# ToughStoneX/Self-Supervised-MVS

Hardware: AMD Instinct MI355X
Metric: depth-samples/sec (N=3, 640x512, D=192) (higher is better)
Workload: dtype f32

## Files before the change

### self-supervised-mvs_amd/_lib.py

```python
from __future__ import annotations

import contextlib
import ctypes as C
import os

_HERE = os.path.dirname(os.path.abspath(__file__))
LIB_PATH = os.path.join(_HERE, "libmvs_hip.so")

_f = C.c_void_p
_i = C.c_int
_ll = C.c_longlong
_s = C.c_void_p
_fl = C.c_float

class MvsUnetBlock(C.Structure):
    _fields_ = [("transposed", _i), ("stride", _i), ("src", _i), ("skip", _i), ("eps", _fl), ("momentum", _fl),
                ("cin", _i), ("cout", _i), ("d", _i), ("h", _i), ("w", _i)]


class MvsFeatBlock(C.Structure):
    _fields_ = [("cin", _i), ("cout", _i), ("ks", _i), ("stride", _i), ("eps", _fl), ("momentum", _fl), ("w_channels_last", _i),
                ("h", _i), ("w", _i)]


# ... 110 lines not shown
    "mvs_maxpool2x2_cl": (_i, [_f, _f, _i, _i, _i, _i, _s]),
    "mvs_resize_bilinear_cl": (_i, [_f, _f, _i, _i, _i, _i, _i, _i, _s]),
    "mvs_conv_trunk_fwd": (_i, [_i, C.POINTER(MvsTrunkLayer), _pp, _pp, _f, _f, _f, _f, _f, _i, _i, _i, _s]),
    "mvs_conv2d_wide_packed_bytes_arith": (_ll, [_i, _i, _i]),
    "mvs_conv2d_wide_workspace_floats_arith": (_ll, [_i] * 6),
    "mvs_conv2d_wide_pack_weights_arith": (_i, [_f, _f, _i, _i, _i, _i, _s]),
    "mvs_conv2d_wide_fwd_arith": (_i, [_f, _f, _f, _f, _f, _i, _i, _i, _i, _i, _i, _i, _i, _s]),
    "mvs_conv_trunk_fwd_arith": (_i, [_i, C.POINTER(MvsTrunkLayer), _pp, _pp, _f, _f, _f, _f, _f, _i, _i, _i, _i, _s]),
}

OP_CONV_FWD, OP_CONV_DGRAD, OP_CONV_WGRAD, OP_CONVT_FWD, OP_CONVT_DGRAD, OP_CONVT_WGRAD = range(6)


class MvsLib:

    def __init__(self, path: str = LIB_PATH, device_type: str = "cuda"):
        if not os.path.exists(path):
            raise RuntimeError(
                "libmvs_hip.so not found at %s -- build it with `python __graft_entry__.py` "
                "(hipcc --offload-arch=gfx950); there is no CPU / PyTorch fallback for the hot path" % path)
        self.path = path
        self.device_type = device_type
        self.cdll = C.CDLL(path)
        self.profiler = None
        for name, (res, args) in SIGNATURES.items():
            fn = getattr(self.cdll, name)
            fn.restype = res
            fn.argtypes = args
            setattr(self, "_" + name, fn)

    def call(self, name: str, *args, tag="", tstream=None):
        prof = self.profiler
        if prof is not None and (prof.names is None or name in prof.names):
            if not isinstance(tag, str):
                tag = tag[0] % tuple(tag[1:])
            if prof.wants(name, tag):
                import torch
                ev0, ev1 = torch.cuda.Event(enable_timing=True), torch.cuda.Event(enable_timing=True)
                ev0.record(tstream)
                rc = getattr(self, "_" + name)(*args)
                ev1.record(tstream)
                prof.add(name, tag, ev0, ev1)
                if rc != 0:
                    self._raise(name, rc)
                return
        rc = getattr(self, "_" + name)(*args)
        if rc != 0:
            self._raise(name, rc)

    def _raise(self, name, rc):
        msg = self._mvs_last_error().decode("utf-8", "replace")
        if rc in (-1, -2, -4):
            raise ValueError("%s failed (%d): %s" % (name, rc, msg))
        raise RuntimeError("%s failed (%d): %s" % (name, rc, msg))

    def raw(self, name: str, *args):
        return getattr(self, "_" + name)(*args)

    def launch_trace(self):
        buf = C.create_string_buffer(4096)
        self._mvs_launch_trace(buf, len(buf))
        return [s for s in buf.value.decode().split(",") if s]

    def get_tuning(self, key: str) -> int:
        v = _i()
        self.call("mvs_get_tuning", key.encode(), C.byref(v))
        return v.value

    @contextlib.contextmanager
    def tuning(self, **knobs):
        old = []
        try:
            for key, val in knobs.items():
                old.append((key, self.get_tuning(key)))
                self.call("mvs_set_tuning", key.encode(), int(val))
            yield self
        finally:
            for key, val in reversed(old):
                self.call("mvs_set_tuning", key.encode(), val)


_INSTANCE = None

DEFAULT_TUNING = {"k8": 7, "xcd": 1, "side_pre": 1, "conv_pers": 1, "conv_pers_min": 1024, "conv_pers_nw": 8, "wgrad_pers": 1, "conv_small": 1, "tr2pw": 1, "sweep_bwd": 0, "wgrad_small": 0, "wgrad_groups": 768, "wgrad8_groups": 192, "wgrad8_gs": 2, "wgrad8_nch": 2, "cout1_h4": 1, "wgrad2d_batch": 2048, "sweep_fwd": 3}


def get() -> MvsLib:
    global _INSTANCE
    if _INSTANCE is None:
        _INSTANCE = MvsLib()
        for item in filter(None, os.environ.get("MVS_TUNING", "").split(",")):
            key, _, val = item.partition("=")
            DEFAULT_TUNING[key.strip()] = int(val)
            _INSTANCE.call("mvs_set_tuning", key.strip().encode(), int(val))
    return _INSTANCE


class KernelTimer:

    def __init__(self, only=None, names=None):
        self.only = only
        self.names = names
        self.events = {}

    def wants(self, name, tag):
        return self.only is None or name in self.only or tag in self.only

    def add(self, name, tag, ev0, ev1):
        self.events.setdefault((name, tag), []).append((ev0, ev1))

    _REG_NAMES = frozenset(("mvs_conv3d_fwd", "mvs_convT3d_fwd", "mvs_conv3d_dgrad", "mvs_convT3d_dgrad", "mvs_conv3d_wgrad", "mvs_convT3d_wgrad",
                            "mvs_bn_relu_fwd_slots", "mvs_bn_relu_bwd_slots", "mvs_bn_bwd_reduce_slots", "mvs_conv3d_pack_weights_batch"))

    def allows_c_entry(self, lib, blocks):
        if self.names is None:
            return False
        hit = self.names & self._REG_NAMES
        if not hit:
            return True
        if not hit <= {"mvs_conv3d_wgrad", "mvs_convT3d_wgrad"} or self.only is None:
            return False
        want = [t for t in self.only if isinstance(t, str) and t.startswith("wgrad")]
        found = []
        for i, (transposed, cin, cout, stride, dims) in enumerate(blocks):
            tag = "%s:%d>%d:s%d:%dx%dx%dx%d" % (("wgradT" if transposed else "wgrad", cin, cout, stride) + tuple(dims))
            if tag in want:
                found.append((i, "mvs_convT3d_wgrad" if transposed else "mvs_conv3d_wgrad", tag))
        if len(found) != 1 or len(want) != 1:
            return False
        owner = getattr(lib, "_unet_timer", None)
        if owner is not self:
            if owner is not None:
                owner._harvest()
                owner._c = None
            lib.raw("mvs_unet_time_read", (C.c_float * 1024)(), 1024)
            lib.raw("mvs_unet_time_wgrad", found[0][0])
            lib._unet_timer = self
            self._c = (lib, found[0])
        return True

    def _harvest(self):
        c = getattr(self, "_c", None)
        if c is None:
            return
        lib, (idx, name, tag) = c
        buf = (C.c_float * 1024)()
        cnt = lib.raw("mvs_unet_time_read", buf, 1024)
        if cnt > 0:
            acc = self.__dict__.setdefault("_c_acc", {})
            n0, s0 = acc.get((name, tag), (0, 0.0))
            acc[(name, tag)] = (n0 + cnt, s0 + sum(buf[:cnt]))

    def release_c_bracket(self, lib):
        self._harvest()
        self._c = None
        lib.raw("mvs_unet_time_wgrad", -2)
        lib._unet_timer = None

    def summary(self):
        out = {}
        for k, evs in self.events.items():
            ms = [a.elapsed_time(b) for a, b in evs]
            out[k] = (len(ms), sum(ms) / len(ms))
        c = getattr(self, "_c", None)
        if c is not None:
            self.release_c_bracket(c[0])
        for (name, tag), (cnt, tot) in getattr(self, "_c_acc", {}).items():
# ... 7 lines not shown
```

### self-supervised-mvs_amd/csrc/conv3d.hip

```cpp
#include "mvs_rt.h"
#include "conv_map.h"

#include "conv_args.h"

__device__ __forceinline__ void conv_pack_weights_item(const float* __restrict__ w, float* __restrict__ wp, int geom, int CC,
                                                       int Cin, int Cout, int NB, int layout, int flip, int idx) {
    const int j = idx & 3, lane = (idx >> 2) & 63;
    const int nb = (idx >> 8) % NB, kk = (idx >> 8) / NB;
    const int co = nb * 16 + (lane & 15);
    int ks, chunk = 0, cls = 0;
    if (geom == GEOM_TR2_PW) {
        int k0 = 0;
        for (cls = 0; cls < 4; ++cls) {
            int n = tr2p_ntaps(cls) * CC / 16;
            if (kk < k0 + n) break;
            k0 += n;
        }
        ks = kk - k0;
        const int kf = 16 * ks + 4 * (lane >> 4) + j;
        const int tp = kf / CC, cip = kf % CC, n = lane & 15, pw = n >> 3, cop = n & 7;
        int dd, dh, dw, kd, kh;
        tr2p_tap(cls, tp, dd, dh, dw, kd, kh);
        int kw = tr2p_kw(pw, dw);
        float v = 0.f;
// ... 968 lines not shown
                acc[p][0] = mfma_4x4x1_bc(w0, x4.x, acc[p][0], 4 * cq + 0);
                acc[p][1] = mfma_4x4x1_bc(w1, x4.x, acc[p][1], 4 * cq + 0);
                acc[p][0] = mfma_4x4x1_bc(w0, x4.y, acc[p][0], 4 * cq + 1);
                acc[p][1] = mfma_4x4x1_bc(w1, x4.y, acc[p][1], 4 * cq + 1);
                acc[p][0] = mfma_4x4x1_bc(w0, x4.z, acc[p][0], 4 * cq + 2);
                acc[p][1] = mfma_4x4x1_bc(w1, x4.z, acc[p][1], 4 * cq + 2);
                acc[p][0] = mfma_4x4x1_bc(w0, x4.w, acc[p][0], 4 * cq + 3);
                acc[p][1] = mfma_4x4x1_bc(w1, x4.w, acc[p][1], 4 * cq + 3);
            }
        }
    }
    const int qd = qd0 + wave, qh = qh0 + (lane >> 4), qw = qw0 + (lane & 15);
    const bool inside = qd < a.QD && qh < a.QH && qw < a.QW;
#pragma unroll
    for (int h = 0; h < 2; ++h) {
        float o[4];
#pragma unroll
        for (int r = 0; r < 4; ++r) {
            const int co = 4 * h + r;
            float val = acc[0][h][r] + acc[1][h][r];
            if (!inside || co >= a.Cout) val = 0.f;
            s1[co] += val;
            s2[co] += val * val;
            if (co < a.Cout) {
                if (a.scale) val = val * a.scale[co] + a.shift[co];
                else if (a.shift) val = val + a.shift[co];
                if (a.relu) val = fmaxf(val, 0.f);
            }
            o[r] = val;
        }
        if (inside) {
            const size_t obase = ((((size_t)b * a.Do + qd) * a.Ho + qh) * a.Wo + qw) * a.Cout + 4 * h;
            if (a.Cout == 8) {
                float4 ov = make_float4(o[0], o[1], o[2], o[3]);
                if (a.skip) {
                    const float4 sk = *reinterpret_cast<const float4*>(a.skip + obase);
                    ov.x += sk.x; ov.y += sk.y; ov.z += sk.z; ov.w += sk.w;
                }
                *reinterpret_cast<float4*>(a.y + obase) = ov;
            } else {
#pragma unroll
                for (int r = 0; r < 4; ++r)
                    if (4 * h + r < a.Cout) a.y[obase + r] = o[r] + (a.skip ? a.skip[obase + r] : 0.f);
            }
        }
    }
    }
    if (a.slots) {
        float v[16];
#pragma unroll
        for (int c = 0; c < 8; ++c) { v[c] = s1[c]; v[8 + c] = s2[c]; }
#define MVS_BFLY_STEP(N, M)                                              \
        {                                                                \
            const bool up = (lane & (M)) != 0;                           \
            _Pragma("unroll") for (int q = 0; q < (N); ++q) {            \
                const float keep = up ? v[(N) + q] : v[q];               \
                const float send = up ? v[q] : v[(N) + q];               \
                v[q] = keep + __shfl_xor(send, (M));                     \
            }                                                            \
        }
        MVS_BFLY_STEP(8, 32)
        MVS_BFLY_STEP(4, 16)
        MVS_BFLY_STEP(2, 8)
        MVS_BFLY_STEP(1, 4)
#undef MVS_BFLY_STEP
        float r = v[0];
        r += __shfl_xor(r, 2);
        r += __shfl_xor(r, 1);
        if ((lane & 3) == 0) {
            const int idx = ((lane >> 5) & 1) * 8 + ((lane >> 4) & 1) * 4 + ((lane >> 3) & 1) * 2 + ((lane >> 2) & 1);
            red[wave * 16 + idx] = r;
        }
        __syncthreads();
        if (tid < 16) {
            const int stat = tid >> 3, co = tid & 7;
            if (co < a.Cout)
                MVS_GLOBAL_ATOMIC_ADD_F64(a.slots + ((size_t)(blockIdx.x & (a.nslots - 1)) * 2 + stat) * a.Cout + co,
                                          (double)(red[tid] + red[16 + tid] + red[32 + tid] + red[48 + tid]));
        }
    }
}


template <bool BC, int NCH>
__global__ __launch_bounds__(256) void conv_c8_wgrad_kernel(WgradArgs a) {
    using G = ConvGeom<GEOM_S1>;
    constexpr int CC = 16, CCP = 16;
    constexpr int RHP = 7, RWP = 19;
    constexpr int NRP = G::RD * RHP * RWP;
    constexpr int NPOS = G::TQD * G::TQH * G::TQW;
    constexpr int NTG = 7;
    __shared__ __attribute__((aligned(16))) float xt[NCH * NRP * CCP];
    __shared__ __attribute__((aligned(16))) float gt[NPOS * 8];
    __shared__ int tapmap[32];
    __shared__ int tapoff[32];
    const int tid = threadIdx.x, lane = tid & 63, wave = tid >> 6;
    const int chunk0 = blockIdx.y * NCH;
    if (tid == 0) {
        int ne = 0, no = 0;
        int ev[16], od[16];
        for (int t = 0; t < 27; ++t) {
            if (((t / 9) + (t / 3) % 3 + t % 3) & 1) od[no++] = t; else ev[ne++] = t;
        }
        od[no++] = 27;
        for (int tg = 0; tg < NTG; ++tg)
            for (int grp = 0; grp < 4; ++grp) {
                const int t = (grp & 1) ? od[2 * tg + (grp >> 1)] : ev[2 * tg + (grp >> 1)];
                const int tt = t < 27 ? t : od[0];
                tapmap[4 * tg + grp] = t;
                tapoff[4 * tg + grp] = (((tt / 9) * RHP + (tt / 3) % 3) * RWP + tt % 3) * CCP;
            }
    }
    __syncthreads();
    int toff[NTG];
#pragma unroll
    for (int tg = 0; tg < NTG; ++tg) toff[tg] = tapoff[4 * tg + (lane >> 4)] + (lane & 15);
    f32x4 acc[NCH][NTG][2];
#pragma unroll
    for (int ch = 0; ch < NCH; ++ch)
#pragma unroll
        for (int tg = 0; tg < NTG; ++tg) { acc[ch][tg][0] = (f32x4){0.f, 0.f, 0.f, 0.f}; acc[ch][tg][1] = (f32x4){0.f, 0.f, 0.f, 0.f}; }

    const int ntiles = a.B * a.ntd * a.nth * a.ntw;
    constexpr int NXI = G::RD * G::RH * G::RW * (CC / 4);
    constexpr int XIT = (NXI + 255) / 256, GIT = (NPOS * 2 + 255) / 256;
    float4 xv[NCH][XIT], gv[GIT];
    int xrel[XIT], xlo[XIT], grel[GIT], glo[GIT];
#pragma unroll
    for (int k = 0; k < XIT; ++k) {
        const int i = tid + 256 * k, vox = i / (CC / 4), cq = i % (CC / 4);
        const int rw = vox % G::RW, rh = (vox / G::RW) % G::RH, rd = vox / (G::RW * G::RH);
        xrel[k] = (((rd - 1) * a.Hi + (rh - 1)) * a.Wi + (rw - 1)) * a.CX + 4 * cq;
        xlo[k] = ((rd * RHP + rh) * RWP + rw) * CCP + 4 * cq;
    }
#pragma unroll
    for (int k = 0; k < GIT; ++k) {
        const int i = tid + 256 * k, p = i >> 1, hq = i & 1;
        const int pw = p % G::TQW, ph = (p / G::TQW) % G::TQH, pd = p / (G::TQW * G::TQH);
        grel[k] = ((pd * a.QH + ph) * a.QW + pw) * 8 + 4 * hq;
        glo[k] = p * 8 + 4 * hq;
    }
    auto load_tile = [&](int tile) {
        int b, td, th, tw;
        if (a.xcd) brick_tile(tile, a.ntw, a.nth, a.ntd, b, td, th, tw);
        else linear_tile(tile, a.ntw, a.nth, a.ntd, b, td, th, tw);
        const int qd0 = td * G::TQD, qh0 = th * G::TQH, qw0 = tw * G::TQW;
        const float* __restrict__ xb = a.x + ((((size_t)b * a.Di + qd0) * a.Hi + qh0) * a.Wi + qw0) * a.CX + chunk0 * CC;
        const float* __restrict__ gb = a.g + ((((size_t)b * a.QD + qd0) * a.QH + qh0) * a.QW + qw0) * 8;
        const bool interior = qd0 >= 1 && qd0 + G::TQD + 1 <= a.Di && qh0 >= 1 && qh0 + G::TQH + 1 <= a.Hi &&
                              qw0 >= 1 && qw0 + G::TQW + 1 <= a.Wi;
        if (interior) {
#pragma unroll
            for (int ch = 0; ch < NCH; ++ch)
#pragma unroll
                for (int k = 0; k < XIT; ++k)
                    if (tid + 256 * k < NXI) xv[ch][k] = *reinterpret_cast<const float4*>(xb + ch * CC + xrel[k]);
#pragma unroll
            for (int k = 0; k < GIT; ++k)
                if (tid + 256 * k < NPOS * 2) gv[k] = *reinterpret_cast<const float4*>(gb + grel[k]);
        } else {
#pragma unroll
            for (int k = 0; k < XIT; ++k) {
                const int i = tid + 256 * k, vox = i / (CC / 4);
                const int rw = vox % G::RW, rh = (vox / G::RW) % G::RH, rd = vox / (G::RW * G::RH);
                const int id = qd0 + rd - 1, ih = qh0 + rh - 1, iw = qw0 + rw - 1;
                const bool in = i < NXI && id >= 0 && id < a.Di && ih >= 0 && ih < a.Hi && iw >= 0 && iw < a.Wi;
// ... 237 lines not shown
        case MVS_OP_CONVT_FWD:
            p.wlayout = WL_IOK; p.Di = D; p.Hi = H; p.Wi = W; p.cin = Cin; p.cout = Cout;
            if (stride == 1) { p.geom = GEOM_S1; p.flip = 1; } else { p.geom = GEOM_TR2; p.flip = 0; }
            return MVS_OK;
        case MVS_OP_CONVT_DGRAD:
            p.wlayout = WL_OIK; p.flip = 0; p.cin = Cout; p.cout = Cin;
            if (stride == 1) { p.geom = GEOM_S1; p.Di = D; p.Hi = H; p.Wi = W; }
            else { p.geom = GEOM_S2; p.Di = 2 * D; p.Hi = 2 * H; p.Wi = 2 * W; }
            return MVS_OK;
        default:
            mvs_set_error("%s: op %d has no weight image", what, op);
            return MVS_ERR_UNSUPPORTED;
    }
}

static void plan_grid(const IgemmPlan& p, int& QD, int& QH, int& QW) {
    if (p.geom == GEOM_S2) { QD = (p.Di - 1) / 2 + 1; QH = (p.Hi - 1) / 2 + 1; QW = (p.Wi - 1) / 2 + 1; }
    else { QD = p.Di; QH = p.Hi; QW = p.Wi; }
}
static bool plan_is_c8(const IgemmPlan& p, const Epilogue* ep) {
    return (g_tune.k8 & 3) && p.geom == GEOM_S1 && p.cout == 8 && (p.cin == 8 || p.cin == 16 || p.cin == 32) && !(ep && ep->bn_raw);
}
static bool plan_is_cout1(const IgemmPlan& p, const Epilogue* ep) {
    return p.geom == GEOM_S1 && p.cout == 1 && p.wlayout == WL_OIK && !p.flip && (p.cin == 8 || p.cin == 16) &&
           !(ep && (ep->slots || ep->bn_raw));
}

static int plan_pack(const IgemmPlan& p, const float* w, float* ws, PackItem& it) {
    it = {};
    it.w = w; it.wp = ws; it.kind = -1;
    if (p.cin1) {
        MVS_REQUIRE(p.cout == 8 || p.cout == 16, MVS_ERR_UNSUPPORTED, "conv3d_dgrad(Cout=1): Cin must be 8 or 16, got %d", p.cout);
        it.kind = 1; it.Cout = p.cout; it.total = 27 * p.cout;
        return MVS_OK;
    }
    MVS_REQUIRE(p.cin == 8 || p.cin == 16 || p.cin == 32 || p.cin == 64, MVS_ERR_UNSUPPORTED,
                "conv igemm: input channels must be 8/16/32/64, got %d", p.cin);
    MVS_REQUIRE(p.cout >= 1 && p.cout <= 64, MVS_ERR_UNSUPPORTED, "conv igemm: output channels must be <= 64, got %d", p.cout);
    MVS_REQUIRE(!(p.geom == GEOM_TR2 && p.cin < 16), MVS_ERR_UNSUPPORTED, "transposed stride-2 conv needs >= 16 input channels");
    int QD, QH, QW, kgeom, NB, nblocks;
    plan_grid(p, QD, QH, QW);
    igemm_tiling(p.geom, p.B, QD, QH, QW, p.cout, kgeom, NB, nblocks);
    const int cc = pick_cc_k(p.geom, kgeom, p.cin);
    const int nb_total = mvs_cdiv(p.cout, 16) == 3 ? 4 : mvs_cdiv(p.cout, 16);
    const int pgeom = (kgeom == GEOM_TR2 && cc == 16 && p.cout == 8 && g_tune.tr2pw) ? GEOM_TR2_PW : p.geom;
    it.kind = 0; it.geom = pgeom; it.CC = cc; it.Cin = p.cin; it.Cout = p.cout; it.NB = nb_total; it.layout = p.wlayout; it.flip = p.flip;
    it.total = (int)((size_t)total_ksteps(pgeom, p.cin, cc) * nb_total * 256);
    return MVS_OK;
}

static int launch_pack(const PackItem* items, int n, hipStream_t st) {
    for (int i0 = 0; i0 < n; i0 += MVS_PACK_BATCH_MAX) {
        PackBatch pb = {};
        int m = 0, maxtotal = 0;
        for (int i = i0; i < n && m < MVS_PACK_BATCH_MAX; ++i) {
            if (items[i].kind < 0) continue;
            pb.it[m++] = items[i];
            if (items[i].total > maxtotal) maxtotal = items[i].total;
        }
        if (m == 0) continue;
        MVS_LAUNCH(conv_pack_batch_kernel, dim3(mvs_cdiv(maxtotal, 256), m), dim3(256), 0, st, pb);
    }
    return mvs_check_launch("conv_pack_weights");
}

static int run_igemm(const IgemmPlan& p, const float* in, const float* wsrc, float* out, float* ws, const Epilogue& ep,
                     int ws_packed, hipStream_t st) {
    MVS_REQUIRE(in && wsrc && out && ws, MVS_ERR_NULL, "conv: null pointer argument");
    MVS_REQUIRE(!ep.slots || (ep.nslots >= 1 && ep.nslots <= 256 && (ep.nslots & (ep.nslots - 1)) == 0), MVS_ERR_SHAPE,
                "conv: statistic slot count must be a power of two <= 256, got %d", ep.nslots);
    MVS_REQUIRE(!ep.bn_raw || (ep.bn_stats && ep.slots), MVS_ERR_NULL, "conv: bn_raw needs bn_stats and slots");
    const int geom = p.geom, B = p.B, cin = p.cin, cout = p.cout;
    ConvArgs a = {};
    a.x = in; a.y = out; a.B = B; a.Di = p.Di; a.Hi = p.Hi; a.Wi = p.Wi; a.Cin = cin; a.Cout = cout;
    a.scale = ep.scale; a.shift = ep.shift; a.skip = ep.skip; a.relu = ep.relu;
    a.slots = ep.slots; a.nslots = ep.nslots; a.bn_raw = ep.bn_raw; a.bn_stats = ep.bn_stats;
    plan_grid(p, a.QD, a.QH, a.QW);
    if (geom == GEOM_S1) { a.Do = p.Di; a.Ho = p.Hi; a.Wo = p.Wi; }
    else if (geom == GEOM_S2) { a.Do = a.QD; a.Ho = a.QH; a.Wo = a.QW; }
    else { a.Do = 2 * p.Di; a.Ho = 2 * p.Hi; a.Wo = 2 * p.Wi; }
    a.ntd = mvs_cdiv(a.QD, geom_tqd(geom)); a.nth = mvs_cdiv(a.QH, geom_tqh(geom)); a.ntw = mvs_cdiv(a.QW, 16);
    if ((g_tune.conv0_x3 & 1) && conv_x3_serves(geom, a)) return run_conv_x3(a, wsrc, p.wlayout, p.flip, st);
    if ((g_tune.conv0_x3 & 2) && conv_x3_fwd_serves(geom, a)) return run_conv_x3_fwd(a, wsrc, p.wlayout, p.flip, ws, st);
    if (plan_is_c8(p, &ep)) {
        const int ntl = B * a.ntd * a.nth * a.ntw;
        const int nbc = ntl < 512 ? ntl : 512;
        if (cin == 32) MVS_LAUNCH((conv_c8_fwd_bc_kernel<16, 2>), dim3(nbc), dim3(256), 0, st, a, wsrc, p.wlayout, p.flip, g_tune.xcd);
        else if (cin == 16) MVS_LAUNCH((conv_c8_fwd_bc_kernel<16, 1>), dim3(nbc), dim3(256), 0, st, a, wsrc, p.wlayout, p.flip, g_tune.xcd);
        else MVS_LAUNCH((conv_c8_fwd_bc_kernel<8, 1>), dim3(nbc), dim3(256), 0, st, a, wsrc, p.wlayout, p.flip, g_tune.xcd);
        return mvs_check_launch("conv_c8_fwd_bc");
    }
    int nblocks = B * a.ntd * a.nth * a.ntw;
    if (plan_is_cout1(p, &ep)) {
        if (cin == 8 && g_tune.cout1_h4) {
            a.ntd = mvs_cdiv(a.QD, CO1_TD); a.nth = mvs_cdiv(a.QH, CO1_TH); a.ntw = mvs_cdiv(a.QW, CO1_TW);
            MVS_LAUNCH(conv_cout1_h4_kernel, dim3(B * a.ntd * a.nth * a.ntw), dim3(256), 0, st, a, wsrc);
        } else if (cin == 8) MVS_LAUNCH((conv_cout1_kernel<8>), dim3(nblocks), dim3(256), 0, st, a, wsrc);
        else MVS_LAUNCH((conv_cout1_kernel<16>), dim3(nblocks), dim3(256), 0, st, a, wsrc);
        return mvs_check_launch(cin == 8 ? (g_tune.cout1_h4 ? "conv_cout1 h4" : "conv_cout1 cin=8") : "conv_cout1 cin=16");
    }
    int NB, kgeom;
    a.nb_total = mvs_cdiv(cout, 16) == 3 ? 4 : mvs_cdiv(cout, 16);
    igemm_tiling(geom, B, a.QD, a.QH, a.QW, cout, kgeom, NB, nblocks);
    const int cc = pick_cc_k(geom, kgeom, cin);
    a.ntd = mvs_cdiv(a.QD, geom_tqd(kgeom)); a.nth = mvs_cdiv(a.QH, geom_tqh(kgeom));
    if (!ws_packed) {
        PackItem it;
        int rc = plan_pack(p, wsrc, ws, it);
        if (rc) return rc;
        rc = launch_pack(&it, 1, st);
        if (rc) return rc;
    } else {
        MVS_REQUIRE(cin == 8 || cin == 16 || cin == 32 || cin == 64, MVS_ERR_UNSUPPORTED, "conv igemm: input channels must be 8/16/32/64, got %d", cin);
        MVS_REQUIRE(cout >= 1 && cout <= 64, MVS_ERR_UNSUPPORTED, "conv igemm: output channels must be <= 64, got %d", cout);
        MVS_REQUIRE(!(geom == GEOM_TR2 && cin < 16), MVS_ERR_UNSUPPORTED, "transposed stride-2 conv needs >= 16 input channels");
    }
    a.wp = ws;
    if (g_tune.conv_pers && conv_pers_serves(geom, cin, cout) && (long)nblocks * (a.nb_total / NB) >= g_tune.conv_pers_min) {
        a.ntd = mvs_cdiv(a.QD, geom_tqd(geom)); a.nth = mvs_cdiv(a.QH, geom_tqh(geom));
        return run_conv_pers(geom, a, st);
    }
    if ((g_tune.conv_pers & 1) && kgeom == GEOM_TR2 && cc == 16 && cout == 8 && g_tune.tr2pw && conv_pers_serves(GEOM_TR2_PW, cin, cout) &&
        nblocks >= g_tune.conv_pers_min)
        return run_conv_pers(GEOM_TR2_PW, a, st);
    if (kgeom == GEOM_S1) return cc == 16 ? launch_igemm_nb<GEOM_S1, 16>(a, NB, nblocks, st)
                                          : launch_igemm_nb<GEOM_S1, 8>(a, NB, nblocks, st);
    if (kgeom == GEOM_S2) return launch_igemm_nb<GEOM_S2, 8>(a, NB, nblocks, st);
    if (kgeom == GEOM_S1_SMALL) {
        if (cc == 64) return launch_igemm_nb<GEOM_S1_SMALL, 64>(a, NB, nblocks, st);
        if (cc == 32) return launch_igemm_nb<GEOM_S1_SMALL, 32>(a, NB, nblocks, st);
        return cc == 16 ? launch_igemm_nb<GEOM_S1_SMALL, 16>(a, NB, nblocks, st) : launch_igemm_nb<GEOM_S1_SMALL, 8>(a, NB, nblocks, st);
    }
    if (kgeom == GEOM_S2_SMALL) {
        if (cc == 32) return launch_igemm_nb<GEOM_S2_SMALL, 32>(a, NB, nblocks, st);
        if (cc == 16) return launch_igemm_nb<GEOM_S2_SMALL, 16>(a, NB, nblocks, st);
        return launch_igemm_nb<GEOM_S2_SMALL, 8>(a, NB, nblocks, st);
    }
    if (kgeom == GEOM_TR2_SMALL) {
        if (cc == 16) return launch_igemm_nb<GEOM_TR2_SMALL, 16>(a, NB, nblocks, st);
        if (cc == 32) return launch_igemm_nb<GEOM_TR2_SMALL, 32>(a, NB, nblocks, st);
        return launch_igemm_nb<GEOM_TR2_SMALL, 64>(a, NB, nblocks, st);
    }
    if (cc == 16 && cout == 8 && g_tune.tr2pw) return launch_igemm_nb<GEOM_TR2_PW, 16>(a, NB, nblocks, st);
    if (cc == 16) return launch_igemm_nb<GEOM_TR2, 16>(a, NB, nblocks, st);
    if (cc == 32) return launch_igemm_nb<GEOM_TR2, 32>(a, NB, nblocks, st);
    return launch_igemm_nb<GEOM_TR2, 64>(a, NB, nblocks, st);
}

static int run_cin1(const IgemmPlan& p, const float* gy, const float* w, float* gx, float* ws, const Epilogue& ep, int ws_packed,
                    hipStream_t st) {
    MVS_REQUIRE(gy && w && gx && ws, MVS_ERR_NULL, "conv3d_dgrad: null pointer argument");
    MVS_REQUIRE(!ep.skip, MVS_ERR_UNSUPPORTED, "conv3d_dgrad: the Cout = 1 input gradient takes no summand");
    MVS_REQUIRE(!ep.bn_raw || (ep.bn_stats && ep.slots), MVS_ERR_NULL, "conv3d_dgrad: bn_raw needs bn_stats and slots");
    MVS_REQUIRE(!ep.slots || (ep.bn_raw && ep.nslots >= 1 && ep.nslots <= 256 && (ep.nslots & (ep.nslots - 1)) == 0), MVS_ERR_SHAPE,
                "conv3d_dgrad: bad statistic slots");
    const int C = p.cout;
    if (!ws_packed) {
        PackItem it;
        int rc = plan_pack(p, w, ws, it);
        if (rc) return rc;
        rc = launch_pack(&it, 1, st);
        if (rc) return rc;
    } else {
        MVS_REQUIRE(C == 8 || C == 16, MVS_ERR_UNSUPPORTED, "conv3d_dgrad(Cout=1): Cin must be 8 or 16, got %d", C);
    }
    const size_t total = (size_t)p.B * p.Di * p.Hi * p.Wi;
// ... 209 lines not shown
```

### self-supervised-mvs_amd/csrc/tuning.h

```cpp
#pragma once

#define MVS_KNOBS(X) \
     \
    X(nt,               0,    0, 1,       "forward: non-temporal stores of the variance volume") \
    X(tile_w,           0,    0, 256,     "cached forward: pixel-tile width, 0 = the default tile") \
    X(dslab,            0,    0, 1 << 20, "forward: planes per workgroup, 0 = auto") \
    X(sweep_fwd,        3,    0, 4,       "forward: 0 taps through L1 every plane, 1 LDS-staged windows, 2 register-cached taps (4 ch/thread), 3 (8 ch/thread), 4 (16 ch/thread, <= 2 source views)") \
    X(sweep_bwd,        0,    0, 1,       "backward: 0 per-wave windows (<= 4 source views), 1 view-pair kernel with LDS atomics (what > 4 source views run)") \
    X(bwd_dslab,        0,    0, 1 << 20, "per-wave-window backward: planes per workgroup, 0 = auto") \
    X(bwd_nowin,        0,    0, 1,       "(tests) 1 = no LDS windows, every flush through global atomics") \
    X(bwd_cpt,          4,    4, 8,       "accepted and ignored (the 8-channels-per-thread backward was measured slower and removed)") \
    X(bwd_pf,           0,    0, 2,       "backward: 1 = block lookahead for 1-2 source views, 2 = ONE wave per SIMD for 3-4 source views") \
    X(bwd_gd,           2,    0, 2,       "backward: 2 = upstream gradient requested two planes ahead at 2 waves/SIMD (1-2 source views), 0 = rotating set at 3 waves/SIMD") \
    X(bwd_gd34,         0,    0, 1,       "backward: 3-4 source views with the upstream gradient requested two planes ahead (as 1-2 views run), 2 waves/SIMD") \
    X(fwd_pt,           0,    0, 1,       "cached forward with the per-wave projection table (plane_sweep_variance_fwd_pt_kernel): measured and rejected") \
    X(bwd_gpf,          0,    0, 1,       "per-wave-window backward requests the next planes' upstream gradient: 0 top of the group, 1 after the plane's gathers") \
    X(fwd_dl,           2,    0, 2,       "forward: 0 the round-1 loop, 1 LDS-staged per-plane depths, 2 + all views' re-gathers in flight before the first sample") \
    X(sweep_xcd,        0,    0, 1,       "XCD-compact workgroup order of the cached forward and the per-wave-window backward") \
     \
    X(conv_split,       1,    0, 1,       "0 keeps all Cout tiles in one workgroup") \
    X(conv_small,       1,    0, 2,       "quarter-size workgroup tiles for under-filled launches (0 never, 1 auto, 2 always)") \
    X(conv_small_wgs,   384,  0, 1 << 20, "... below this many workgroups (~1.5 per CU)") \
    X(tr2pw,            1,    0, 1,       "transposed stride-2 conv with Cout == 8 as W-parity-merged GEMMs (GEOM_TR2_PW)") \
    X(cc_wide,          0,    0, 1,       "quarter-tile kernels of the deep levels with all input channels as one chunk: measured and rejected") \
    X(cin1_vpt,         1,    1, 5,       "voxels per thread of the Cout == 1 layer's input gradient (4 = four from 1 M voxels on, 5 = always four): measured and rejected") \
    X(k8,               7,    0, 15,      "bit mask: 1|2 = Cout == 8 stride-1 layers run the 4x4x1 MFMA forward with the weights as the broadcast operand (0: generic kernel), +4 = weight gradient with g as the broadcast operand") \
    X(cout1_d4,         2,    0, 3,       "bit 1: the Cout = 1 layer of the bf16 inference path with four outputs per thread") \
    X(cout1_h4,         1,    0, 1,       "the 8 -> 1 layer with four outputs per thread (conv_cout1_h4_kernel); 0: one output per thread") \
    X(bf16_dp,          1,    0, 1,       "conv0 of the bf16 path (32 -> 8) with two output depth slices per MFMA (GEOM_S1_DP)") \
    X(xcd,              1,    0, 1,       "XCD-aware tile order in the broadcast-operand forward and the Cout == 8 weight gradient") \
    X(side_pre,         1,    0, 1,       "one-Cout-tile kernels with epilogue side inputs (skip / bn_raw) request them before the k-loop (1) or at the top of the epilogue (0)") \
    X(conv_pers,        1,    0, 1,       "one-chunk layers (16 -> <= 16, 8 -> 32 stride 1; 8 -> <= 16 stride 2) run the persistent kernels of conv3d_pers.hip") \
    X(conv_pers_min,    1024, 0, 1 << 30, "... when the one-tile kernel would launch at least this many workgroups (a persistent grid needs several tiles per workgroup)") \
    X(conv_pers_groups, 0,    0, 4096,    "workgroups of a persistent launch, 0 = what fits the GPU (tests: a few workgroups walk many tiles)") \
    X(conv_pers_nw,     8,    4, 8,       "waves per workgroup of conv_pers_kernel") \
    X(wgrad_pers,       1,    0, 1,       "one-chunk weight gradients run conv3d_pers.hip, from conv_pers_min tiles on") \
    X(wgrad_small,      0,    0, 3,       "quarter-size tiles in the generic weight-gradient kernel: 1 = 8-channel / stride-2 layers with many tiles, 2 = every layer with many tiles, 3 = always (tests)") \
    X(wgrad_groups,     768,  1, 768,     "persistent workgroups of the generic weight-gradient kernels") \
    X(wgrad8_groups,    192,  1, 512,     "... of the CG == 8 kernel (conv0)") \
    X(wgrad8_gs,        2,    0, 2,       "conv0's weight gradient in the output-gradient-shifted form on the 16x16x4 MFMA (conv_c8_wgrad_gs_kernel): 1 eight waves per workgroup, 2 sixteen; 0: conv_c8_wgrad_kernel (4x4x1 MFMA, X shifted)") \
    X(wgrad8_nch,       2,    1, 2,       "2 = the CG == 8 weight gradient stages both 16-channel chunks of a 32-channel X in one workgroup") \
    X(conv0_x3,         0,    0, 3,       "split-bf16 products (conv3d_x3.hip, opt-in): bit 0 = conv0's input gradient, bit 1 = conv0's forward") \
     \
    X(conv2d_pp,        1,    0, 1,       "3x3 stride-1 layers with <= 8 output channels as pixel-pair GEMMs (conv2d_igemm_kernel<.., PP>)") \
    X(conv2d_s2_mfma,   2,    0, 2,       "stride-2 input gradient: 2 ONE four-class MFMA pass with compacted taps, 1 four parity-class passes, 0 direct VALU form") \
    X(wgrad2d_groups,   256,  0, 1 << 20, "persistent workgroups of the weight gradient (used: 1 .. 1024; 256 = one per CU)") \
    X(wgrad2d_batch,    2048, 1, 4096,    "workgroups of the batched weight gradient (both launches together), shared out by work") \
     \
    X(c2w_tile,         0,    0, 2,       "0 = t128x64 when its launch has at least c2w_big_min workgroups, else t64x64; 1 = always t64x64; 2 = always t128x64") \
    X(c2w_big_min,      512,  0, 1 << 30, "... workgroups (two per CU)") \
    X(c2w_splitk,       0,    0, 8,       "K ranges of a layer: 0 = doubled (<= 8) while a t64x64 launch has fewer than c2w_split_min workgroups, 1 = never split, 2..8 = this many") \
    X(c2w_split_min,    512,  0, 1 << 30, "... workgroups (two per CU)") \
    X(c2w_bf_split_min, 2048, 0, 1 << 30, "c2w_split_min of the bf16 arms (arith = bf16): eight workgroups per CU")

struct MvsTuning {
#define MVS_KNOB_FIELD(key, def, lo, hi, doc) int key;
    MVS_KNOBS(MVS_KNOB_FIELD)
#undef MVS_KNOB_FIELD
};
extern MvsTuning g_tune;
```

Before: 212.8.

## Run conv0 forward as Winograd F(2,3) along depth on fp32 MFMA

Adds a persistent forward kernel for the 32->8 channel conv0 layer that applies a Winograd F(2,3) transform along the depth axis. Input planes are transformed while being staged into LDS, weights are pre-transformed per block, and the output is recovered with an inverse transform after a cross-wave exchange. This cuts the multiply count along depth from three taps to two per output pair, and it prefetches the next chunk or tile into registers during compute. In exchange it pays for the transforms, extra LDS traffic and register pressure, and the transformed arithmetic may change fp32 rounding slightly.

```diff
diff --git a/self-supervised-mvs_amd/_lib.py b/self-supervised-mvs_amd/_lib.py
--- a/self-supervised-mvs_amd/_lib.py
+++ b/self-supervised-mvs_amd/_lib.py
@@ -216,7 +216,7 @@
 
 _INSTANCE = None
 
-DEFAULT_TUNING = {"k8": 7, "xcd": 1, "side_pre": 1, "conv_pers": 1, "conv_pers_min": 1024, "conv_pers_nw": 8, "wgrad_pers": 1, "conv_small": 1, "tr2pw": 1, "sweep_bwd": 0, "wgrad_small": 0, "wgrad_groups": 768, "wgrad8_groups": 192, "wgrad8_gs": 2, "wgrad8_nch": 2, "cout1_h4": 1, "wgrad2d_batch": 2048, "sweep_fwd": 3}
+DEFAULT_TUNING = {"k8": 7, "xcd": 1, "side_pre": 1, "conv_pers": 1, "conv_pers_min": 1024, "conv_pers_nw": 8, "wgrad_pers": 1, "conv_small": 1, "tr2pw": 1, "sweep_bwd": 0, "wgrad_small": 0, "wgrad_groups": 768, "wgrad8_groups": 192, "wgrad8_gs": 2, "wgrad8_nch": 2, "cout1_h4": 1, "wgrad2d_batch": 2048, "sweep_fwd": 3, "conv0_wino": 1}
 
 
 def get() -> MvsLib:
diff --git a/self-supervised-mvs_amd/csrc/conv3d.hip b/self-supervised-mvs_amd/csrc/conv3d.hip
--- a/self-supervised-mvs_amd/csrc/conv3d.hip
+++ b/self-supervised-mvs_amd/csrc/conv3d.hip
@@ -1074,6 +1074,8 @@
 }
 
 
+#include "conv3d_wino_kernels.h"
+
 template <bool BC, int NCH>
 __global__ __launch_bounds__(256) void conv_c8_wgrad_kernel(WgradArgs a) {
     using G = ConvGeom<GEOM_S1>;
@@ -1477,6 +1479,13 @@
     a.ntd = mvs_cdiv(a.QD, geom_tqd(geom)); a.nth = mvs_cdiv(a.QH, geom_tqh(geom)); a.ntw = mvs_cdiv(a.QW, 16);
     if ((g_tune.conv0_x3 & 1) && conv_x3_serves(geom, a)) return run_conv_x3(a, wsrc, p.wlayout, p.flip, st);
     if ((g_tune.conv0_x3 & 2) && conv_x3_fwd_serves(geom, a)) return run_conv_x3_fwd(a, wsrc, p.wlayout, p.flip, ws, st);
+    if (g_tune.conv0_wino && plan_is_c8(p, &ep) && cin == 32 &&
+        (g_tune.conv0_wino == 2 || (long)B * a.ntd * a.nth * a.ntw >= 1024)) {
+        const int ntl = B * a.ntd * a.nth * a.ntw;
+        const int groups = g_tune.conv_pers_groups > 0 ? g_tune.conv_pers_groups : 512;
+        MVS_LAUNCH(conv_c8_fwd_bc_kernel_wino, dim3(ntl < groups ? ntl : groups), dim3(256), 0, st, a, wsrc, p.wlayout, p.flip, g_tune.xcd);
+        return mvs_check_launch("conv_c8_fwd_wino");
+    }
     if (plan_is_c8(p, &ep)) {
         const int ntl = B * a.ntd * a.nth * a.ntw;
         const int nbc = ntl < 512 ? ntl : 512;
diff --git a/self-supervised-mvs_amd/csrc/conv3d_wino_kernels.h b/self-supervised-mvs_amd/csrc/conv3d_wino_kernels.h
--- /dev/null
+++ b/self-supervised-mvs_amd/csrc/conv3d_wino_kernels.h
@@ -0,0 +1,216 @@
+#pragma once
+
+__global__ __launch_bounds__(256) void conv_c8_fwd_bc_kernel_wino(ConvArgs a, const float* __restrict__ w, int wlayout, int flip, int xcd) {
+    constexpr int TQD = 4, TQH = 4, TQW = 16, NP = TQD / 2;
+    constexpr int RH = TQH + 2, RW = TQW + 2, HW = RH * RW;
+    constexpr int CC = 8, NCH = 4, NT = 256;
+    constexpr int ROWW = RW * CC + 4, PLW = RH * ROWW;
+    __shared__ __attribute__((aligned(16))) float tile[NP * 4 * PLW];
+    __shared__ float wl[2 * 9 * 4 * 2 * 64];
+    static_assert(4 * NT * 4 <= NP * 4 * PLW, "the exchange image lives in the tile");
+    float* xch = tile;
+    __shared__ float red[4 * 8];
+    const int tid = threadIdx.x, lane = tid & 63, wave = tid >> 6;
+    const int pw = wave & 1, cg = wave >> 1;
+    const int ntiles = a.B * a.ntd * a.nth * a.ntw;
+    const int vb = xcd ? xcd_block(blockIdx.x, gridDim.x) : (int)blockIdx.x;
+    const float4* tile4 = reinterpret_cast<const float4*>(tile);
+    const int baseB4 = (pw * 4) * (PLW / 4) + (lane >> 4) * (ROWW / 4) + (lane & 15) * (CC / 4) + cg;
+    const int wlane = (lane + 16 * cg) & 63;
+
+    auto tile_origin = [&](int t, int& b, int& qd0, int& qh0, int& qw0) {
+        int td, th, tw;
+        if (xcd) brick_tile(t, a.ntw, a.nth, a.ntd, b, td, th, tw);
+        else linear_tile(t, a.ntw, a.nth, a.ntd, b, td, th, tw);
+        qd0 = td * TQD; qh0 = th * TQH; qw0 = tw * TQW;
+    };
+    constexpr int NI = NP * HW * 2, XIT = (NI + NT - 1) / NT;
+    float4 xv[XIT][4];
+    int rel[XIT], sdst[XIT];
+    const int pstep = a.Hi * a.Wi * a.Cin;
+#pragma unroll
+    for (int k = 0; k < XIT; ++k) {
+        const int i = tid + NT * k, c4 = i & 1, hw = (i >> 1) % HW, p = (i >> 1) / HW;
+        const int rh = hw / RW, rw = hw % RW;
+        rel[k] = (((2 * p - 1) * a.Hi + (rh - 1)) * a.Wi + (rw - 1)) * a.Cin + 4 * c4;
+        sdst[k] = (p * 4) * PLW + rh * ROWW + rw * CC + 4 * c4;
+    }
+    auto load_chunk = [&](int b, int qd0, int qh0, int qw0, int chunk) {
+        const float* __restrict__ base = a.x + ((((size_t)b * a.Di + qd0) * a.Hi + qh0) * a.Wi + qw0) * a.Cin + chunk * CC;
+        const bool interior = qd0 >= 1 && qd0 + TQD + 1 <= a.Di && qh0 >= 1 && qh0 + TQH + 1 <= a.Hi &&
+                              qw0 >= 1 && qw0 + TQW + 1 <= a.Wi;
+        if (interior) {
+#pragma unroll
+            for (int k = 0; k < XIT; ++k)
+                if (tid + NT * k < NI) {
+#pragma unroll
+                    for (int pl = 0; pl < 4; ++pl) xv[k][pl] = *reinterpret_cast<const float4*>(base + rel[k] + pl * pstep);
+                }
+        } else {
+#pragma unroll
+            for (int k = 0; k < XIT; ++k) {
+                const int i = tid + NT * k, hw = (i >> 1) % HW, p = (i >> 1) / HW;
+                const int ih = qh0 + hw / RW - 1, iw = qw0 + hw % RW - 1;
+                const bool in_hw = i < NI && ih >= 0 && ih < a.Hi && iw >= 0 && iw < a.Wi;
+#pragma unroll
+                for (int pl = 0; pl < 4; ++pl) {
+                    const int id = qd0 + 2 * p + pl - 1;
+                    xv[k][pl] = make_float4(0.f, 0.f, 0.f, 0.f);
+                    if (in_hw && id >= 0 && id < a.Di) xv[k][pl] = *reinterpret_cast<const float4*>(base + rel[k] + pl * pstep);
+                }
+            }
+        }
+    };
+    auto store_chunk = [&]() {
+#pragma unroll
+        for (int k = 0; k < XIT; ++k) {
+            if (tid + NT * k < NI) {
+                const float4 d0 = xv[k][0], d1 = xv[k][1], d2 = xv[k][2], d3 = xv[k][3];
+                float* dst = &tile[sdst[k]];
+                *reinterpret_cast<float4*>(dst) = make_float4(d0.x - d2.x, d0.y - d2.y, d0.z - d2.z, d0.w - d2.w);
+                *reinterpret_cast<float4*>(dst + PLW) = make_float4(d1.x + d2.x, d1.y + d2.y, d1.z + d2.z, d1.w + d2.w);
+                *reinterpret_cast<float4*>(dst + 2 * PLW) = make_float4(d2.x - d1.x, d2.y - d1.y, d2.z - d1.z, d2.w - d1.w);
+                *reinterpret_cast<float4*>(dst + 3 * PLW) = make_float4(d1.x - d3.x, d1.y - d3.y, d1.z - d3.z, d1.w - d3.w);
+            }
+        }
+    };
+    int b, qd0, qh0, qw0;
+    if (vb < ntiles) {
+        tile_origin(vb, b, qd0, qh0, qw0);
+        load_chunk(b, qd0, qh0, qw0, 0);
+    }
+    for (int i = tid; i < 2 * 9 * 4 * 2 * 64; i += NT) {
+        const int l = i & 63, h = (i >> 6) & 1, j = (i >> 7) & 3, t9 = (i >> 9) % 9, ch = (i >> 9) / 9;
+        const int ci = ch * 16 + (l >> 2), co = 4 * h + (l & 3);
+        float g[3];
+#pragma unroll
+        for (int kd = 0; kd < 3; ++kd) {
+            const int tap = kd * 9 + t9, kidx = flip ? 26 - tap : tap;
+            g[kd] = wlayout == WL_OIK ? w[((size_t)co * a.Cin + ci) * 27 + kidx] : w[((size_t)ci * a.Cout + co) * 27 + kidx];
+        }
+        float v = g[0];
+        if (j == 1) v = ((g[0] + g[1]) + g[2]) * 0.5f;
+        else if (j == 2) v = ((g[0] - g[1]) + g[2]) * 0.5f;
+        else if (j == 3) v = g[2];
+        wl[i] = v;
+    }
+    float s1[4], s2[4];
+#pragma unroll
+    for (int c = 0; c < 4; ++c) { s1[c] = 0.f; s2[c] = 0.f; }
+    for (int t = vb; t < ntiles; t += gridDim.x) {
+    tile_origin(t, b, qd0, qh0, qw0);
+    f32x4 acc[4][2];
+#pragma unroll
+    for (int j = 0; j < 4; ++j) { acc[j][0] = (f32x4){0.f, 0.f, 0.f, 0.f}; acc[j][1] = (f32x4){0.f, 0.f, 0.f, 0.f}; }
+
+#pragma unroll
+    for (int ch = 0; ch < NCH; ++ch) {
+        __syncthreads();
+        store_chunk();
+        __syncthreads();
+        if (ch + 1 < NCH) load_chunk(b, qd0, qh0, qw0, ch + 1);
+        else if (t + (int)gridDim.x < ntiles) {
+            int b2, d2, h2, w2;
+            tile_origin(t + gridDim.x, b2, d2, h2, w2);
+            load_chunk(b2, d2, h2, w2, 0);
+        }
+        float4 xq[2][4];
+        float wq[2][4][2];
+        auto read_tap = [&](int t9, float4 (&dst)[4], float (&wd)[4][2]) {
+            const int toff4 = (t9 / 3) * (ROWW / 4) + (t9 % 3) * (CC / 4);
+#pragma unroll
+            for (int j = 0; j < 4; ++j) {
+                dst[j] = tile4[baseB4 + j * (PLW / 4) + toff4];
+                wd[j][0] = wl[((((ch >> 1) * 9 + t9) * 4 + j) * 2 + 0) * 64 + wlane];
+                wd[j][1] = wl[((((ch >> 1) * 9 + t9) * 4 + j) * 2 + 1) * 64 + wlane];
+            }
+        };
+        read_tap(0, xq[0], wq[0]);
+#pragma unroll
+        for (int t9 = 0; t9 < 9; ++t9) {
+            if (t9 + 1 < 9) read_tap(t9 + 1, xq[(t9 + 1) & 1], wq[(t9 + 1) & 1]);
+            MVS_SCHED_FENCE();
+            const int s = t9 & 1;
+            const float tj[4][4] = {{xq[s][0].x, xq[s][0].y, xq[s][0].z, xq[s][0].w}, {xq[s][1].x, xq[s][1].y, xq[s][1].z, xq[s][1].w},
+                                    {xq[s][2].x, xq[s][2].y, xq[s][2].z, xq[s][2].w}, {xq[s][3].x, xq[s][3].y, xq[s][3].z, xq[s][3].w}};
+#pragma unroll
+            for (int e = 0; e < 4; ++e) {
+#pragma unroll
+                for (int j = 0; j < 4; ++j) {
+                    acc[j][0] = mfma_4x4x1_bc(wq[s][j][0], tj[j][e], acc[j][0], 8 * (ch & 1) + e);
+                    acc[j][1] = mfma_4x4x1_bc(wq[s][j][1], tj[j][e], acc[j][1], 8 * (ch & 1) + e);
+                }
+            }
+        }
+    }
+    __syncthreads();
+#pragma unroll
+    for (int j = 0; j < 4; ++j)
+        *reinterpret_cast<f32x4*>(&xch[(j * NT + tid) * 4]) = cg ? acc[j][0] : acc[j][1];
+    __syncthreads();
+    f32x4 m[4];
+#pragma unroll
+    for (int j = 0; j < 4; ++j) {
+        const f32x4 other = *reinterpret_cast<const f32x4*>(&xch[(j * NT + (tid ^ 128)) * 4]);
+        const f32x4 mine = cg ? acc[j][1] : acc[j][0];
+        m[j] = mine + other;
+    }
+    const f32x4 out[2] = {(m[0] + m[1]) + m[2], (m[1] - m[2]) - m[3]};
+    const int qh = qh0 + (lane >> 4), qw = qw0 + (lane & 15);
+#pragma unroll
+    for (int u = 0; u < 2; ++u) {
+        const int qd = qd0 + 2 * pw + u;
+        const bool inside = qd < a.QD && qh < a.QH && qw < a.QW;
+        float o[4];
+#pragma unroll
+        for (int r = 0; r < 4; ++r) {
+            const int co = 4 * cg + r;
+            float val = inside ? out[u][r] : 0.f;
+            s1[r] += val;
+            s2[r] += val * val;
+            if (a.scale) val = val * a.scale[co] + a.shift[co];
+            else if (a.shift) val = val + a.shift[co];
+            if (a.relu) val = fmaxf(val, 0.f);
+            o[r] = val;
+        }
+        if (inside) {
+            const size_t obase = ((((size_t)b * a.Do + qd) * a.Ho + qh) * a.Wo + qw) * 8 + 4 * cg;
+            float4 ov = make_float4(o[0], o[1], o[2], o[3]);
+            if (a.skip) {
+                const float4 sk = *reinterpret_cast<const float4*>(a.skip + obase);
+                ov.x += sk.x; ov.y += sk.y; ov.z += sk.z; ov.w += sk.w;
+            }
+            *reinterpret_cast<float4*>(a.y + obase) = ov;
+        }
+    }
+    }
+    if (a.slots) {
+        float v[8];
+#pragma unroll
+        for (int c = 0; c < 4; ++c) { v[c] = s1[c]; v[4 + c] = s2[c]; }
+#define MVS_BFLY_STEP(N, M)                                              \
+        {                                                                \
+            const bool up = (lane & (M)) != 0;                           \
+            _Pragma("unroll") for (int q = 0; q < (N); ++q) {            \
+                const float keep = up ? v[(N) + q] : v[q];               \
+                const float send = up ? v[q] : v[(N) + q];               \
+                v[q] = keep + __shfl_xor(send, (M));                     \
+            }                                                            \
+        }
+        MVS_BFLY_STEP(4, 32)
+        MVS_BFLY_STEP(2, 16)
+        MVS_BFLY_STEP(1, 8)
+#undef MVS_BFLY_STEP
+        float r = v[0];
+        r += __shfl_xor(r, 4);
+        r += __shfl_xor(r, 2);
+        r += __shfl_xor(r, 1);
+        if ((lane & 7) == 0) red[wave * 8 + ((lane >> 5) & 1) * 4 + ((lane >> 4) & 1) * 2 + ((lane >> 3) & 1)] = r;
+        __syncthreads();
+        if (tid < 16) {
+            const int stat = tid >> 3, co = tid & 7, wv = 2 * (co >> 2), idx = stat * 4 + (co & 3);
+            MVS_GLOBAL_ATOMIC_ADD_F64(a.slots + ((size_t)(blockIdx.x & (a.nslots - 1)) * 2 + stat) * 8 + co,
+                                      (double)(red[wv * 8 + idx] + red[(wv + 1) * 8 + idx]));
+        }
+    }
+}
diff --git a/self-supervised-mvs_amd/csrc/tuning.h b/self-supervised-mvs_amd/csrc/tuning.h
--- a/self-supervised-mvs_amd/csrc/tuning.h
+++ b/self-supervised-mvs_amd/csrc/tuning.h
@@ -41,6 +41,7 @@
     X(wgrad8_gs,        2,    0, 2,       "conv0's weight gradient in the output-gradient-shifted form on the 16x16x4 MFMA (conv_c8_wgrad_gs_kernel): 1 eight waves per workgroup, 2 sixteen; 0: conv_c8_wgrad_kernel (4x4x1 MFMA, X shifted)") \
     X(wgrad8_nch,       2,    1, 2,       "2 = the CG == 8 weight gradient stages both 16-channel chunks of a 32-channel X in one workgroup") \
     X(conv0_x3,         0,    0, 3,       "split-bf16 products (conv3d_x3.hip, opt-in): bit 0 = conv0's input gradient, bit 1 = conv0's forward") \
+    X(conv0_wino,       1,    0, 2,       "conv0's forward (32 -> 8) as Winograd F(2,3) along D on the fp32 MFMA (conv3d_wino_kernels.h): 0 never, 1 from 1024 tiles of the 4x4x16 grid on, 2 always (tests)") \
      \
     X(conv2d_pp,        1,    0, 1,       "3x3 stride-1 layers with <= 8 output channels as pixel-pair GEMMs (conv2d_igemm_kernel<.., PP>)") \
     X(conv2d_s2_mfma,   2,    0, 2,       "stride-2 input gradient: 2 ONE four-class MFMA pass with compacted taps, 1 four parity-class passes, 0 direct VALU form") \
```

Measured after the change: 214.6, median of 6. About the same (+0.9%).
